# rpng/suo_slam

Hardware: AMD Instinct MI355X
Metric: frames/sec (obj-crops/sec) YCB-V 640x480 8-obj; ADD(-S) vs ref (higher is better)
Workload: dtype f32 (2 x fp16 split products)

## Files before the change

### suo_slam_amd/csrc/conv_wino_x3.hip

```cpp
#include <string.h>

#include "bf16x3.h"
#include "f16x2.h"
#include "buffer_ops.h"
#include "suo_internal.h"
#include "tune.h"

namespace suo {

typedef float x_f32x4 __attribute__((ext_vector_type(4)));
typedef float x_f32x16 __attribute__((ext_vector_type(16)));
typedef unsigned x_u32x2 __attribute__((ext_vector_type(2)));
typedef unsigned x_u32x4 __attribute__((ext_vector_type(4)));
typedef __bf16 x_bf16x8 __attribute__((ext_vector_type(8)));
typedef _Float16 x_f16x8 __attribute__((ext_vector_type(8)));

__device__ __forceinline__ x_f32x16 x_mfma32(float a, float b, x_f32x16 c) { return __builtin_amdgcn_mfma_f32_32x32x2f32(a, b, c, 0, 0, 0); }
__device__ __forceinline__ int x_acc_row(int r, int lane) { return (r & 3) + 8 * (r >> 2) + 4 * (lane >> 5); }

__device__ __forceinline__ x_f32x4 x_sub4(x_f32x4 a, x_f32x4 b) { return a - b; }
__device__ __forceinline__ x_f32x4 x_add4(x_f32x4 a, x_f32x4 b) { return a + b; }
__device__ __forceinline__ void x_add16(x_f32x16& z, const x_f32x16& t) { z += t; }
__device__ __forceinline__ void x_sub16(x_f32x16& z, const x_f32x16& t) { z -= t; }

constexpr int X_CK = 16, X_PKH = 20, X_TH = 8, X_TW = 16, X_IH = 10, X_IW = 18, X_NPIX = X_IH * X_IW;

void pack_wino_weight_bf16x3(const float* W, int N, int C, int Np, int Cp, const float* out_scale, uint16_t* out) {
    static const double G[4][3] = {{1, 0, 0}, {0.5, 0.5, 0.5}, {0.5, -0.5, 0.5}, {0, 0, 1}};
    const int NB = Np / 32;
    memset(out, 0, (size_t)Np * Cp * 16 * 3 * sizeof(uint16_t));
    for (int n = 0; n < N; ++n)
        for (int c = 0; c < C; ++c) {
            const float* g = W + ((size_t)n * C + c) * 9;
            const double sc = out_scale ? (double)out_scale[n] : 1.0;
            double Gg[4][3], U[4][4];
            for (int i = 0; i < 4; ++i)
                for (int j = 0; j < 3; ++j) Gg[i][j] = G[i][0] * g[j] + G[i][1] * g[3 + j] + G[i][2] * g[6 + j];
            for (int i = 0; i < 4; ++i)
                for (int j = 0; j < 4; ++j) U[i][j] = (Gg[i][0] * G[j][0] + Gg[i][1] * G[j][1] + Gg[i][2] * G[j][2]) * sc;
            const int chunk = c / X_CK, cc = c % X_CK, nb = n / 32, lane = (cc / 8) * 32 + (n % 32), e = cc % 8;
            for (int comp = 0; comp < 16; ++comp) {
                uint16_t t[3];
                s3_split_host((float)(comp >= 12 ? -U[comp >> 2][comp & 3] : U[comp >> 2][comp & 3]), t);
                for (int p = 0; p < 3; ++p) out[((((size_t)(chunk * 16 + comp) * NB + nb) * 3 + p) * 64 + lane) * 8 + e] = t[p];
            }
        }
}

void pack_tail_weight_bf16x3(const float* W3, int N2, int K, uint16_t* out) {
    const int NB = N2 / 32;
    for (int n = 0; n < N2; ++n)
        for (int k = 0; k < K; ++k) {
            const int ks = k / 16, kk = k % 16, lane = (kk / 8) * 32 + (n % 32), e = kk % 8, nb = n / 32;
            uint16_t t[3];
            s3_split_host(W3[(size_t)n * K + k], t);
            for (int p = 0; p < 3; ++p) out[((((size_t)(ks * NB + nb) * 3 + p) * 64 + lane) * 8) + e] = t[p];
        }
}

void pack_wino_weight_f16x2(const float* W, int N, int C, int Np, int Cp, const float* out_scale, uint16_t* out, float* oscale_out) {
    static const double G[4][3] = {{1, 0, 0}, {0.5, 0.5, 0.5}, {0.5, -0.5, 0.5}, {0, 0, 1}};
    const int NB = Np / 32;
    memset(out, 0, (size_t)Np * Cp * 16 * 2 * sizeof(uint16_t));
    for (int n = 0; n < Np; ++n) oscale_out[n] = ldexpf(1.f, -S2_XSHIFT);
    float* Un = (float*)malloc((size_t)C * 16 * sizeof(float));
    for (int n = 0; n < N; ++n) {
        float mx = 0.f;
        for (int c = 0; c < C; ++c) {
            const float* g = W + ((size_t)n * C + c) * 9;
            const double sc = out_scale ? (double)out_scale[n] : 1.0;
            double Gg[4][3];
            for (int i = 0; i < 4; ++i)
                for (int j = 0; j < 3; ++j) Gg[i][j] = G[i][0] * g[j] + G[i][1] * g[3 + j] + G[i][2] * g[6 + j];
            for (int i = 0; i < 4; ++i)
                for (int j = 0; j < 4; ++j) {
                    const float u = (float)((Gg[i][0] * G[j][0] + Gg[i][1] * G[j][1] + Gg[i][2] * G[j][2]) * sc);
                    Un[c * 16 + i * 4 + j] = i == 3 ? -u : u;
                    mx = fmaxf(mx, fabsf(u));
                }
        }
        const int t = s2_row_shift(mx);
        oscale_out[n] = ldexpf(1.f, -(t + S2_XSHIFT));
        for (int c = 0; c < C; ++c) {
            const int chunk = c / X_CK, cc = c % X_CK, nb = n / 32, lane = (cc / 8) * 32 + (n % 32), e = cc % 8;
            for (int comp = 0; comp < 16; ++comp) {
                uint16_t h[2];
                s2_split_host(ldexpf(Un[c * 16 + comp], t), h);
                for (int p = 0; p < 2; ++p) out[((((size_t)(chunk * 16 + comp) * NB + nb) * 2 + p) * 64 + lane) * 8 + e] = h[p];
            }
        }
    }
    free(Un);
}

void pack_tail_weight_f16x2(const float* W3, int N2, int K, uint16_t* out, float* oscale_out) { pack_gemm_weight_f16x2(W3, N2, K, out, oscale_out); }

template <bool FUSE, bool UP = false, bool TX3 = false, int NT = 4, int NP = 3, bool NEXT = false, bool W8 = false>
__global__ __launch_bounds__(W8 ? 512 : 256) __attribute__((amdgpu_waves_per_eu(2))) void wino3x3_x3_kernel(const ConvArgs a) {
    static_assert(NT == 4 || (NT == 2 && !FUSE), "64-channel form: plain convolution only");
    static_assert(!W8 || (NT == 4 && NP == 2 && !NEXT && (TX3 || !FUSE)), "eight waves: the fp16 form of the 128-channel kernel, without the next block's conv1");
    constexpr int NTHR = W8 ? 512 : 256;
    static_assert(!NEXT || (FUSE && TX3 && NP == 2), "the next block's conv1 rides on the fp16 tail");
    static_assert(NP == 3 || !FUSE || TX3, "the fp16 form's tail runs on the fp16 pipe");
    constexpr int HSZ = X_NPIX * X_PKH;
    constexpr int VROW = 16;
    constexpr int VPL = 16 * 32 * VROW;
    constexpr int VFLOATS = NP * VPL / 2;
    constexpr int TAILF = NP * 8 * (64 * 32 + 32) / 4;
    constexpr int SFLOATS = W8 ? (2 * HSZ + VFLOATS > TAILF + 8 * 32 * 36 ? 2 * HSZ + VFLOATS : TAILF + 8 * 32 * 36) : 2 * HSZ + VFLOATS;
    __shared__ __attribute__((aligned(16))) float S[SFLOATS];
    float (*Hin)[HSZ] = reinterpret_cast<float (*)[HSZ]>(&S[0]);
    uint16_t* V = reinterpret_cast<uint16_t*>(&S[2 * HSZ]);
    const int tid = threadIdx.x, lane = tid & 63;
    const int w = __builtin_amdgcn_readfirstlane(tid >> 6);
    const int tiles_x = (a.OW + X_TW - 1) / X_TW, tiles_y = (a.OH + X_TH - 1) / X_TH;
    int bid = blockIdx.x;
    if ((gridDim.x & 7) == 0) bid = (bid & 7) * (gridDim.x >> 3) + (bid >> 3);
    const int l = bid / (tiles_x * tiles_y);
    bid -= l * tiles_x * tiles_y;
    const int ty0 = bid / tiles_x, tx0 = bid - ty0 * tiles_x;
    const int oy0 = ty0 * X_TH, ox0 = tx0 * X_TW;
    const int iy0 = oy0 - 1, ix0 = ox0 - 1;
    const int nch = a.C / X_CK;
    const float* in_l = a.in + (size_t)l * a.H * a.W * a.C;
    const __amdgpu_buffer_rsrc_t in_srd = make_srd(in_l, (size_t)a.H * a.W * a.C * sizeof(float));
    const __amdgpu_buffer_rsrc_t w_srd = make_srd(a.Wp, (size_t)a.N * a.C * 16 * NP * sizeof(uint16_t));
    const __amdgpu_buffer_rsrc_t out_srd = make_srd(a.out + (size_t)l * a.OH * a.OW * a.N, (size_t)a.OH * a.OW * a.N * sizeof(float));

    constexpr int NF4 = X_NPIX * 4, NLD = (NF4 + NTHR - 1) / NTHR;
    int avoff[NLD];
#pragma unroll
    for (int i = 0; i < NLD; ++i) {
        const int idx = tid + i * NTHR;
        const int pix = idx >> 2, cc = idx & 3;
        const int py = pix / X_IW, px = pix - py * X_IW;
        const int iy = iy0 + py, ix = ix0 + px;
        const bool ok = idx < NF4 && iy >= 0 && iy < a.H && ix >= 0 && ix < a.W;
        avoff[i] = ok ? ((iy * a.W + ix) * a.C + cc * 4) * 4 : BUF_OOB;
    }
    x_f32x4 areg[NLD];
    auto gload = [&](int c) {
#pragma unroll
        for (int i = 0; i < NLD; ++i) areg[i] = buf_load(in_srd, avoff[i], c * X_CK * 4);
    };
    float dmax = 0.f;
    const float xs = NP == 2 ? s2_xscale(a.xscale) : 1.f;
    auto sstore = [&](int buf) {
#pragma unroll
        for (int i = 0; i < NLD; ++i) {
            const int idx = tid + i * NTHR;
            if constexpr (NP == 2) {
                areg[i] *= xs;
                dmax = s2_track(s2_track(dmax, areg[i][0], areg[i][1]), areg[i][2], areg[i][3]);
            }
            if (idx < NF4) *(x_f32x4*)&Hin[buf][(idx >> 2) * X_PKH + (idx & 3) * 4] = areg[i];
        }
    };
    const int wvoff = lane * 16;
    const int wn = NT == 4 ? (W8 ? (w & 3) : w) : (w & 1), wc = NT == 4 ? (W8 ? (w >> 2) : 0) : (w >> 1);
    constexpr bool HALF = NT == 2 || W8;
    constexpr int NPAIR = HALF ? 4 : 8;
    const int wsbase = wn * NP * 1024;
    auto bload = [&](int gc, x_u32x4 (&b)[NP]) {
        const int g = gc;
#pragma unroll
        for (int p = 0; p < NP; ++p) b[p] = __builtin_bit_cast(x_u32x4, buf_load(w_srd, wvoff + p * 1024, g * (NT * NP * 1024) + wsbase));
    };
    const int tt = tid & 31, tq = (tid >> 5) & 3, th = (tid >> 7) & 1;
    const int tv = __builtin_amdgcn_readfirstlane(tid >> 8);
    const int t_ty = tt >> 3, t_tx = tt & 7;
    const int hbase = ((2 * t_ty + th) * X_IW + 2 * t_tx) * X_PKH + tq * 4;
    const int vbase = tt * VROW + ((((tq >> 1) ^ (((tt >> 2) ^ (tt >> 3)) & 1)) * 8) + (tq & 1) * 4);
    auto vstore = [&](int comp, x_f32x4 v) {
        if constexpr (NP == 2) {
            const unsigned h0 = s2_pack_rn(v[0], v[1]), h1 = s2_pack_rn(v[2], v[3]);
            *(x_u32x2*)&V[comp * 32 * VROW + vbase] = x_u32x2{h0, h1};
            const unsigned l0 = s2_lo_pack(v[0], v[1], h0), l1 = s2_lo_pack(v[2], v[3], h1);
            *(x_u32x2*)&V[VPL + comp * 32 * VROW + vbase] = x_u32x2{l0, l1};
            return;
        }
#pragma unroll
        for (int p = 0; p < 3; ++p) {
            const unsigned q0 = s3_pack_rn(v[0], v[1]), q1 = s3_pack_rn(v[2], v[3]);
            *(x_u32x2*)&V[p * VPL + comp * 32 * VROW + vbase] = x_u32x2{q0, q1};
            if (p < 2) {
                v = x_sub4(v, x_f32x4{s3_lo(q0), s3_hi(q0), s3_lo(q1), s3_hi(q1)});
            }
        }
    };
    const int hother = th ? 0 : 2 * X_IW * X_PKH;
    const float hsign = th ? -1.f : 1.f;
    auto transform = [&](int buf) {
        const float* hs = &Hin[buf][hbase];
        if constexpr (W8) {
            const int xi = tv == 0 ? (th ? 3 : 0) : (th ? 2 : 1);
            x_f32x4 e[4];
#pragma unroll
            for (int c = 0; c < 4; ++c) {
                if (tv == 0) {
                    e[c] = x_sub4(*(const x_f32x4*)(hs + c * X_PKH), *(const x_f32x4*)(hs + (2 * X_IW + c) * X_PKH));
                } else {
                    const x_f32x4 l1 = *(const x_f32x4*)(hs + (X_IW + c) * X_PKH), lx = *(const x_f32x4*)(hs + hother + c * X_PKH);
                    e[c] = x_f32x4{__builtin_fmaf(lx[0], hsign, l1[0]), __builtin_fmaf(lx[1], hsign, l1[1]), __builtin_fmaf(lx[2], hsign, l1[2]), __builtin_fmaf(lx[3], hsign, l1[3])};
                }
            }
            vstore(xi * 4 + 0, x_sub4(e[0], e[2]));
            vstore(xi * 4 + 1, x_add4(e[1], e[2]));
            vstore(xi * 4 + 2, x_sub4(e[2], e[1]));
            vstore(xi * 4 + 3, x_sub4(e[1], e[3]));
            return;
        }
        x_f32x4 L0[4], L1[4], L2[4], Lx[4];
#pragma unroll
        for (int c = 0; c < 4; ++c) {
            L0[c] = *(const x_f32x4*)(hs + c * X_PKH);
            L1[c] = *(const x_f32x4*)(hs + (X_IW + c) * X_PKH);
            L2[c] = *(const x_f32x4*)(hs + (2 * X_IW + c) * X_PKH);
            Lx[c] = *(const x_f32x4*)(hs + hother + c * X_PKH);
        }
        x_f32x4 eA[4], eB[4];
#pragma unroll
        for (int c = 0; c < 4; ++c) {
            eA[c] = x_sub4(L0[c], L2[c]);
            eB[c] = x_f32x4{__builtin_fmaf(Lx[c][0], hsign, L1[c][0]), __builtin_fmaf(Lx[c][1], hsign, L1[c][1]), __builtin_fmaf(Lx[c][2], hsign, L1[c][2]),
                            __builtin_fmaf(Lx[c][3], hsign, L1[c][3])};
        }
        const int xiA = th ? 3 : 0, xiB = th ? 2 : 1;
        vstore(xiA * 4 + 0, x_sub4(eA[0], eA[2]));
        vstore(xiA * 4 + 1, x_add4(eA[1], eA[2]));
        vstore(xiA * 4 + 2, x_sub4(eA[2], eA[1]));
        vstore(xiA * 4 + 3, x_sub4(eA[1], eA[3]));
        vstore(xiB * 4 + 0, x_sub4(eB[0], eB[2]));
        vstore(xiB * 4 + 1, x_add4(eB[1], eB[2]));
        vstore(xiB * 4 + 2, x_sub4(eB[2], eB[1]));
        vstore(xiB * 4 + 3, x_sub4(eB[1], eB[3]));
    };

    x_f32x16 zero16;
#pragma unroll
    for (int r = 0; r < 16; ++r) zero16[r] = 0.f;
    x_f32x16 out[4], Z[8];
#pragma unroll
    for (int p = 0; p < 4; ++p)
#pragma unroll
        for (int r = 0; r < 16; ++r) out[p][r] = 0.f;
#pragma unroll
    for (int p = 0; p < 8; ++p)
#pragma unroll
        for (int r = 0; r < 16; ++r) Z[p][r] = 0.f;
    auto mac6 = [&](x_f32x16& acc, const x_bf16x8 (&f)[NP], const x_u32x4 (&bw)[NP], bool from_zero) {
        if constexpr (NP == 2) {
            constexpr int UI[3] = {0, 1, 0}, UJ[3] = {1, 0, 0};
#pragma unroll
            for (int t = 0; t < 3; ++t)
                acc = __builtin_amdgcn_mfma_f32_32x32x16_f16(__builtin_bit_cast(x_f16x8, f[UI[t]]), __builtin_bit_cast(x_f16x8, bw[UJ[t]]), (t == 0 && from_zero) ? zero16 : acc, 0, 0, 0);
            return;
        }
        constexpr int TI[6] = {0, 1, 2, 0, 1, 0}, TJ[6] = {2, 1, 0, 1, 0, 0};
#pragma unroll
        for (int t = 0; t < 6; ++t)
            acc = __builtin_amdgcn_mfma_f32_32x32x16_bf16(f[TI[t] % NP], __builtin_bit_cast(x_bf16x8, bw[TJ[t] % NP]), (t == 0 && from_zero) ? zero16 : acc, 0, 0, 0);
    };
    auto comp_of = [&](int pair, int which) -> int {
        if (!HALF) return pair < 4 ? (which ? 12 + pair : pair) : (which ? 8 + (pair - 4) : 4 + (pair - 4));
        return wc * 8 + 2 * pair + which;
    };
    const int afoff = (lane & 31) * VROW + (((lane >> 5) ^ (((lane >> 2) ^ (lane >> 3)) & 1)) * 8);
    x_u32x4 bring[2][2][NP];
    gload(0);
    bload(comp_of(0, 0), bring[0][0]);
    bload(comp_of(0, 1), bring[0][1]);
    sstore(0);
    __syncthreads();

#ifdef SUO_WX3_PROF
    long long pt[5] = {0, 0, 0, 0, 0}, p0 = clock64();
#define XPROF(i) do { const long long _t = clock64(); pt[i] += _t - p0; p0 = _t; } while (0)
#else
#define XPROF(i) do { } while (0)
#endif
    for (int c = 0; c < nch; ++c) {
        const int buf = c & 1;
        const bool more = c + 1 < nch;
        if (more) gload(c + 1);
        transform(buf);
        XPROF(0);
        __syncthreads();
        XPROF(1);
        if (more) sstore(buf ^ 1);
        XPROF(2);
#pragma unroll
        for (int pair = 0; pair < NPAIR; ++pair) {
            const int slot = pair & 1;
            {
                const int np = pair + 1 < NPAIR ? pair + 1 : 0, nc = pair + 1 < NPAIR ? c : (more ? c + 1 : c);
                bload(nc * 16 + comp_of(np, 0), bring[slot ^ 1][0]);
                bload(nc * 16 + comp_of(np, 1), bring[slot ^ 1][1]);
            }
            const int ca = comp_of(pair, 0), cb = comp_of(pair, 1);
            x_bf16x8 afa[NP], afb[NP];
#pragma unroll
            for (int p = 0; p < NP; ++p) {
                afa[p] = *(const x_bf16x8*)&V[p * VPL + ca * 32 * VROW + afoff];
                afb[p] = *(const x_bf16x8*)&V[p * VPL + cb * 32 * VROW + afoff];
            }
            __builtin_amdgcn_sched_barrier(0);
            if (HALF) {
                mac6(Z[2 * pair], afa, bring[slot][0], false);
                mac6(Z[2 * pair + 1], afb, bring[slot][1], false);
            } else if (pair < 4) {
                mac6(Z[pair], afa, bring[slot][0], false);
                mac6(Z[4 + pair], afb, bring[slot][1], false);
            } else {
                x_f32x16 ta, tb;
                mac6(ta, afa, bring[slot][0], true);
                mac6(tb, afb, bring[slot][1], true);
                x_add16(Z[pair - 4], ta); x_add16(Z[pair - 4], tb); x_add16(Z[pair], ta); x_sub16(Z[pair], tb);
            }
            __builtin_amdgcn_sched_barrier(0);
        }
        XPROF(3);
        __syncthreads();
        XPROF(4);
    }
#ifdef SUO_WX3_PROF
    if (blockIdx.x == 1000 && (tid & 63) == 0) printf("wave %d cycles: transform %lld  barrier1 %lld  sstore %lld  mfma+fold %lld  barrier2 %lld\n", w, pt[0], pt[1], pt[2], pt[3], pt[4]);
#endif
    if constexpr (NP == 2) s2_raise(a.range_flag, 4.f * dmax);
#pragma unroll
    for (int h = 0; h < 2; ++h) {
        out[2 * h] = Z[4 * h] + Z[4 * h + 1] + Z[4 * h + 2];
        out[2 * h + 1] = Z[4 * h + 1] - Z[4 * h + 2] - Z[4 * h + 3];
    }
    x_f32x16 mine[2];
    if constexpr (W8) {
        static_assert(VFLOATS >= 8 * 16 * 64, "the exchange area is the V planes");
        float* X = &S[2 * HSZ];
        const int pw = (1 - wc) * 4 + wn;
#pragma unroll
        for (int q = 0; q < 2; ++q) {
#pragma unroll
            for (int r = 0; r < 16; ++r) X[(w * 16 + r) * 64 + lane] = wc == 0 ? out[2 + q][r] : out[q][r];
            __syncthreads();
#pragma unroll
            for (int r = 0; r < 16; ++r) mine[q][r] = (wc == 0 ? out[q][r] + out[2 + q][r] : out[2 + q][r] - out[q][r]) + X[(pw * 16 + r) * 64 + lane];
            __syncthreads();
        }
    }

    if constexpr (FUSE && TX3) {
        constexpr int KS_STRIDE = 64 * 32 + 32;
        constexpr int PL_STRIDE = 8 * KS_STRIDE;
        static_assert(NP * PL_STRIDE == TAILF * 4 && NP * PL_STRIDE + (W8 ? 8 : 4) * 32 * 36 * 4 <= SFLOATS * 4, "tail staging must fit the workgroup's LDS");
        constexpr int NJ = W8 ? 1 : 2;
        unsigned char* AP = reinterpret_cast<unsigned char*>(&S[0]);
        float* T = &S[NP * PL_STRIDE / 4] + w * (32 * 36);
        const __amdgpu_buffer_rsrc_t w3_srd = make_srd(a.W3p, (size_t)a.N * a.N2 * NP * sizeof(uint16_t));
        const size_t crop2 = (size_t)a.OH * a.OW * a.N2;
        const __amdgpu_buffer_rsrc_t r_srd = make_srd(a.R + (size_t)l * crop2, crop2 * sizeof(float));
        const __amdgpu_buffer_rsrc_t o2_srd = make_srd(a.out2 + (size_t)l * crop2, crop2 * sizeof(float));
        constexpr bool has_up = UP;
        const __amdgpu_buffer_rsrc_t up_srd = make_srd(has_up ? a.up + (size_t)l * (crop2 / 4) : a.R, has_up ? crop2 / 4 * sizeof(float) : 0);
        const float xs3 = NP == 2 ? s2_xscale(a.xscale3) : 1.f;
        const float b2v = NP == 2 ? a.bias[wn * 32 + (lane & 31)] * xs3 : a.bias[wn * 32 + (lane & 31)];
        const float c2v = NP == 2 ? a.oscale[wn * 32 + (lane & 31)] * xs3 : 1.f;
        float tmax = 0.f;
        const int sbase = (2 * wn + ((lane >> 4) & 1)) * KS_STRIDE + (lane >> 5) * (8 * 32) + ((((lane >> 3) & 1) ^ (lane >> 5)) * 16) + (lane & 7) * 2;
        const int aoff = (lane & 31) * 32 + (((lane >> 5) ^ ((lane >> 3) & 1)) * 16);
        const int w3voff = lane * 16;
        auto b3load = [&](int ks, x_u32x4 (&b)[2][NP]) {
            const int k = ks < 8 ? ks : 7;
#pragma unroll
            for (int j = 0; j < NJ; ++j)
#pragma unroll
                for (int p = 0; p < NP; ++p) b[j][p] = __builtin_bit_cast(x_u32x4, buf_load(w3_srd, w3voff, (((k * 8 + (W8 ? w : 4 * j + w)) * NP) + p) * 1024));
        };
#pragma unroll
        for (int h = 0; h < 2; ++h) {
            x_u32x4 b3[2][2][NP];
            b3load(0, b3[0]);
            if (!W8 || wc == h)
#pragma unroll
            for (int pj = 0; pj < 2; ++pj)
#pragma unroll
                for (int r = 0; r < 16; ++r) {
                    const float cv = W8 ? mine[pj][r] : out[2 * h + pj][r];
                    float v = NP == 2 ? fmaxf(fmaf(cv, c2v, b2v), 0.f) : fmaxf(cv + b2v, 0.f);
                    const int off = sbase + (16 * (r >> 2) + 2 * (r & 3) + pj) * 32;
                    if constexpr (NP == 2) {
                        tmax = fmaxf(tmax, v);
                        const _Float16 hi = (_Float16)v, lo = (_Float16)(v - (float)hi);
                        *reinterpret_cast<_Float16*>(AP + off) = hi;
                        *reinterpret_cast<_Float16*>(AP + PL_STRIDE + off) = lo;
                        continue;
                    }
#pragma unroll
                    for (int p = 0; p < 3; ++p) {
                        const unsigned q = s3_pack_rn(v, v);
                        *reinterpret_cast<uint16_t*>(AP + p * PL_STRIDE + off) = (uint16_t)(q >> 16);
                        if (p < 2) v -= s3_hi(q);
                    }
                }
            __syncthreads();
            x_f32x16 acc2[2][2];
#pragma unroll
            for (int i = 0; i < 2; ++i)
#pragma unroll
                for (int j = 0; j < 2; ++j)
#pragma unroll
                    for (int r = 0; r < 16; ++r) acc2[i][j][r] = 0.f;
#pragma unroll
            for (int ks = 0; ks < 8; ++ks) {
                b3load(ks + 1, b3[(ks + 1) & 1]);
                x_bf16x8 af[2][NP];
#pragma unroll
                for (int i = 0; i < 2; ++i)
#pragma unroll
                    for (int p = 0; p < NP; ++p) af[i][p] = *(const x_bf16x8*)(AP + p * PL_STRIDE + ks * KS_STRIDE + i * 1024 + aoff);
                __builtin_amdgcn_sched_barrier(0);
#pragma unroll
                for (int i = 0; i < 2; ++i)
#pragma unroll
                    for (int j = 0; j < NJ; ++j) mac6(acc2[i][j], af[i], b3[ks & 1][j], false);
                __builtin_amdgcn_sched_barrier(0);
            }
            if constexpr (NEXT) __syncthreads();
            x_f32x16 acc1[2];
            if constexpr (NEXT) {
#pragma unroll
                for (int i = 0; i < 2; ++i) acc1[i] = zero16;
            }
#pragma unroll
            for (int j = 0; j < NJ; ++j) {
#pragma unroll
                for (int i = 0; i < 2; ++i) {
                    const int col = (W8 ? w : 4 * j + w) * 32 + (lane & 7) * 4;
                    const x_f32x4 bv = *(const x_f32x4*)(a.bias3 + col);
                    x_f32x4 osc3 = x_f32x4{1.f, 1.f, 1.f, 1.f};
                    if constexpr (NP == 2) osc3 = *(const x_f32x4*)(a.oscale3 + col);
                    x_f32x4 nsc, nsh;
                    if constexpr (NEXT) { const float nxs = s2_xscale(a.n_xscale); nsc = *(const x_f32x4*)(a.n_scale + col) * nxs; nsh = *(const x_f32x4*)(a.n_shift + col) * nxs; }
                    int off[4];
                    x_f32x4 rv[4], uv[UP ? 4 : 1];
#pragma unroll
                    for (int k = 0; k < 4; ++k) {
                        const int m = 32 * i + (lane >> 3) + 8 * k;
                        const int oy = oy0 + 2 * (m >> 4) + h, ox = ox0 + (m & 15);
                        const bool in = oy < a.OH && ox < a.OW;
                        off[k] = in ? ((oy * a.OW + ox) * a.N2 + col) * 4 : BUF_OOB;
                        rv[k] = buf_load(r_srd, off[k], 0);
                        if constexpr (UP && !NEXT) uv[k] = buf_load(up_srd, in ? (((oy >> 1) * (a.OW >> 1) + (ox >> 1)) * a.N2 + col) * 4 : BUF_OOB, 0);
                    }
#pragma unroll
                    for (int r = 0; r < 16; ++r) T[x_acc_row(r, lane) * 36 + (lane & 31)] = acc2[i][j][r];
                    __builtin_amdgcn_wave_barrier();
#pragma unroll
                    for (int k = 0; k < 4; ++k) {
                        if constexpr (UP && NEXT) {
                            const int m = 32 * i + (lane >> 3) + 8 * k;
                            const int oy = oy0 + 2 * (m >> 4) + h, ox = ox0 + (m & 15);
                            uv[0] = buf_load(up_srd, (oy < a.OH && ox < a.OW) ? (((oy >> 1) * (a.OW >> 1) + (ox >> 1)) * a.N2 + col) * 4 : BUF_OOB, 0);
                        }
                        x_f32x4 o = *(const x_f32x4*)&T[((lane >> 3) + 8 * k) * 36 + (lane & 7) * 4];
                        if constexpr (NP == 2) o *= osc3;
                        o = (o + bv) + rv[k];
                        if constexpr (UP) o += uv[NEXT ? 0 : k];
                        buf_store(o, o2_srd, off[k]);
                        if constexpr (NEXT) {
                            const int m = 32 * i + (lane >> 3) + 8 * k;
                            float xn[4];
#pragma unroll
                            for (int c = 0; c < 4; ++c) xn[c] = fmaxf(fmaf(o[c], nsc[c], nsh[c]), 0.f);
                            tmax = fmaxf(fmaxf(tmax, fmaxf(xn[0], xn[1])), fmaxf(xn[2], xn[3]));
                            const unsigned h0 = s2_pack_rn(xn[0], xn[1]), h1 = s2_pack_rn(xn[2], xn[3]);
                            const unsigned l0 = s2_lo_pack(xn[0], xn[1], h0), l1 = s2_lo_pack(xn[2], xn[3], h1);
                            unsigned char* d = AP + (2 * w + ((lane & 7) >> 2)) * KS_STRIDE + m * 32 + (((((lane & 3) >> 1) ^ ((m >> 3) & 1))) * 16) + (lane & 1) * 8;
                            *reinterpret_cast<x_u32x2*>(d) = x_u32x2{h0, h1};
                            *reinterpret_cast<x_u32x2*>(d + PL_STRIDE) = x_u32x2{l0, l1};
                        }
                    }
                    __builtin_amdgcn_wave_barrier();
                }
                if constexpr (NEXT) {
                    const __amdgpu_buffer_rsrc_t n1_srd = make_srd(a.n_W1, (size_t)128 * 256 * 2 * sizeof(uint16_t));
                    auto n1load = [&](int q, x_u32x4 (&b)[2]) {
                        const int ksg = 8 * j + (q < 8 ? q : 7);
#pragma unroll
                        for (int p = 0; p < 2; ++p) b[p] = __builtin_bit_cast(x_u32x4, buf_load(n1_srd, w3voff + p * 1024, ((ksg * 4 + w) * 2) * 1024));
                    };
                    constexpr int NR = 4;
                    x_u32x4 nb[NR][2];
#pragma unroll
                    for (int q = 0; q < NR - 1; ++q) n1load(q, nb[q]);
                    __syncthreads();
#pragma unroll
                    for (int q = 0; q < 8; ++q) {
                        n1load(q + NR - 1, nb[(q + NR - 1) % NR]);
                        x_bf16x8 af[2][2];
#pragma unroll
                        for (int i = 0; i < 2; ++i)
#pragma unroll
                            for (int p = 0; p < 2; ++p) af[i][p] = *(const x_bf16x8*)(AP + p * PL_STRIDE + q * KS_STRIDE + i * 1024 + aoff);
                        __builtin_amdgcn_sched_barrier(0);
#pragma unroll
                        for (int i = 0; i < 2; ++i) mac6(acc1[i], af[i], nb[q % NR], false);
                        __builtin_amdgcn_sched_barrier(0);
                    }
                    __syncthreads();
                }
            }
            if constexpr (NEXT) {
                const int col = w * 32 + (lane & 7) * 4;
                const x_f32x4 b1 = *(const x_f32x4*)(a.n_b1 + col), o1 = *(const x_f32x4*)(a.n_osc1 + col);
                const size_t cropn = (size_t)a.OH * a.OW * 128;
                const __amdgpu_buffer_rsrc_t n_srd = make_srd(a.n_out + (size_t)l * cropn, cropn * sizeof(float));
#pragma unroll
                for (int i = 0; i < 2; ++i) {
#pragma unroll
                    for (int r = 0; r < 16; ++r) T[x_acc_row(r, lane) * 36 + (lane & 31)] = acc1[i][r];
                    __builtin_amdgcn_wave_barrier();
#pragma unroll
                    for (int k = 0; k < 4; ++k) {
                        const int m = 32 * i + (lane >> 3) + 8 * k;
                        const int oy = oy0 + 2 * (m >> 4) + h, ox = ox0 + (m & 15);
                        x_f32x4 o = *(const x_f32x4*)&T[((lane >> 3) + 8 * k) * 36 + (lane & 7) * 4];
                        o *= o1;
                        o += b1;
#pragma unroll
                        for (int c = 0; c < 4; ++c) o[c] = fmaxf(o[c], 0.f);
                        buf_store(o, n_srd, (oy < a.OH && ox < a.OW) ? ((oy * a.OW + ox) * 128 + col) * 4 : BUF_OOB);
                    }
                    __builtin_amdgcn_wave_barrier();
                }
            }
            if (h == 0 && !NEXT) __syncthreads();
        }
        if constexpr (NP == 2) s2_raise(a.range_flag, tmax);
        return;
    }

    if constexpr (FUSE && !TX3) {
        constexpr int MP = 132;
        static_assert(128 * MP <= 2 * HSZ + VFLOATS, "the conv2 tile must fit the workgroup's LDS");
        float* M2 = &S[0];
        const int wm = w >> 1, wn = w & 1;
        const int NB2 = a.N2 >> 5;
        const __amdgpu_buffer_rsrc_t w3_srd = make_srd(a.W3p, (size_t)a.N * a.N2 * sizeof(float));
        const size_t crop2 = (size_t)a.OH * a.OW * a.N2;
        const __amdgpu_buffer_rsrc_t r_srd = make_srd(a.R + (size_t)l * crop2, crop2 * sizeof(float));
        const __amdgpu_buffer_rsrc_t o2_srd = make_srd(a.out2 + (size_t)l * crop2, crop2 * sizeof(float));
        constexpr bool has_up = UP;
        const __amdgpu_buffer_rsrc_t up_srd = make_srd(has_up ? a.up + (size_t)l * (crop2 / 4) : a.R, has_up ? crop2 / 4 * sizeof(float) : 0);
        const float b2v = a.bias[w * 32 + (lane & 31)];
        const int w3voff = lane * 16;
        auto b3load = [&](int q, x_f32x4(&b)[4]) {
            const int kg = q < 16 ? q : 15;
#pragma unroll
            for (int j = 0; j < 4; ++j) b[j] = buf_load(w3_srd, w3voff, (kg * NB2 + wn * 4 + j) * 1024);
        };
        constexpr int R3 = 3;
        x_f32x4 b3[R3][4];
#pragma unroll
        for (int r = 0; r < R3 - 1; ++r) b3load(r, b3[r]);
#pragma unroll
        for (int p = 0; p < 4; ++p)
#pragma unroll
            for (int r = 0; r < 16; ++r) {
                const int t = x_acc_row(r, lane);
                const int pix = (2 * (t >> 3) + (p >> 1)) * X_TW + 2 * (t & 7) + (p & 1);
                M2[pix * MP + w * 32 + (lane & 31)] = fmaxf(out[p][r] + b2v, 0.f);
            }
        __syncthreads();
        x_f32x16 acc2[2][4];
#pragma unroll
        for (int i = 0; i < 2; ++i)
#pragma unroll
            for (int j = 0; j < 4; ++j)
#pragma unroll
                for (int r = 0; r < 16; ++r) acc2[i][j][r] = 0.f;
        const float* ms = M2 + ((wm * 2) * 32 + (lane & 31)) * MP + (lane >> 5) * 4;
#pragma unroll
        for (int q = 0; q < 16; ++q) {
            b3load(q + R3 - 1, b3[(q + R3 - 1) % R3]);
            __builtin_amdgcn_sched_barrier(0);
            x_f32x4 af[2];
#pragma unroll
            for (int i = 0; i < 2; ++i) af[i] = *(const x_f32x4*)(ms + i * 32 * MP + q * 8);
#pragma unroll
            for (int t = 0; t < 4; ++t)
#pragma unroll
                for (int i = 0; i < 2; ++i)
#pragma unroll
                    for (int j = 0; j < 4; ++j) acc2[i][j] = x_mfma32(af[i][t], b3[q % R3][j][t], acc2[i][j]);
            __builtin_amdgcn_sched_barrier(0);
        }
        __syncthreads();
#pragma unroll
        for (int i = 0; i < 2; ++i)
#pragma unroll
            for (int j = 0; j < 4; ++j) {
                float* T = M2 + w * (32 * 36);
                const int col = (wn * 4 + j) * 32 + (lane & 7) * 4;
                const x_f32x4 bv = *(const x_f32x4*)(a.bias3 + col);
                int off[4];
                x_f32x4 rv[4], uv[UP ? 4 : 1];
#pragma unroll
                for (int k = 0; k < 4; ++k) {
                    const int pp = (wm * 2 + i) * 32 + (lane >> 3) + 8 * k;
                    const int oy = oy0 + pp / X_TW, ox = ox0 + pp % X_TW;
                    const bool in = oy < a.OH && ox < a.OW;
                    off[k] = in ? ((oy * a.OW + ox) * a.N2 + col) * 4 : BUF_OOB;
                    rv[k] = buf_load(r_srd, off[k], 0);
                    if constexpr (UP) uv[k] = buf_load(up_srd, in ? (((oy >> 1) * (a.OW >> 1) + (ox >> 1)) * a.N2 + col) * 4 : BUF_OOB, 0);
                }
#pragma unroll
                for (int r = 0; r < 16; ++r) T[x_acc_row(r, lane) * 36 + (lane & 31)] = acc2[i][j][r];
                __builtin_amdgcn_wave_barrier();
#pragma unroll
                for (int k = 0; k < 4; ++k) {
                    x_f32x4 o = (*(const x_f32x4*)&T[((lane >> 3) + 8 * k) * 36 + (lane & 7) * 4] + bv) + rv[k];
                    if constexpr (UP) o += uv[k];
                    buf_store(o, o2_srd, off[k]);
                }
                __builtin_amdgcn_wave_barrier();
            }
        return;
    }

    if constexpr (NT == 2 || W8) {
        if constexpr (NT == 2) {
            float* X = &S[2 * HSZ];
#pragma unroll
            for (int q = 0; q < 2; ++q)
#pragma unroll
                for (int r = 0; r < 16; ++r) X[((w * 2 + q) * 16 + r) * 64 + lane] = wc == 0 ? out[2 + q][r] : out[q][r];
            __syncthreads();
            const int pw = (1 - wc) * 2 + wn;
#pragma unroll
            for (int q = 0; q < 2; ++q)
#pragma unroll
                for (int r = 0; r < 16; ++r)
                    mine[q][r] = (wc == 0 ? out[q][r] + out[2 + q][r] : out[2 + q][r] - out[q][r]) + X[((pw * 2 + q) * 16 + r) * 64 + lane];
            __syncthreads();
        }
        float* T = &S[2 * HSZ] + w * (32 * 36);
        const int col = wn * 32 + (lane & 7) * 4;
        const x_f32x4 bv = *(const x_f32x4*)(a.bias + col);
        x_f32x4 osc = x_f32x4{1.f, 1.f, 1.f, 1.f};
        if constexpr (NP == 2) osc = *(const x_f32x4*)(a.oscale + col);
#pragma unroll
        for (int q = 0; q < 2; ++q) {
            const int p = 2 * wc + q, pi = p >> 1, pj = p & 1;
#pragma unroll
            for (int r = 0; r < 16; ++r) T[x_acc_row(r, lane) * 36 + (lane & 31)] = mine[q][r];
            __builtin_amdgcn_wave_barrier();
#pragma unroll
            for (int k = 0; k < 4; ++k) {
                const int t = (lane >> 3) + 8 * k;
                const int oy = oy0 + 2 * (t >> 3) + pi, ox = ox0 + 2 * (t & 7) + pj;
                x_f32x4 o = *(const x_f32x4*)&T[t * 36 + (lane & 7) * 4];
                if constexpr (NP == 2) o *= osc;
                o += bv;
                if (a.relu) {
#pragma unroll
                    for (int z = 0; z < 4; ++z) o[z] = fmaxf(o[z], 0.f);
                }
                buf_store(o, out_srd, (oy < a.OH && ox < a.OW) ? ((oy * a.OW + ox) * a.N + col) * 4 : BUF_OOB);
            }
            __builtin_amdgcn_wave_barrier();
        }
        return;
    }

    float* T = &S[2 * HSZ] + w * (32 * 36);
    const int col = w * 32 + (lane & 7) * 4;
    const x_f32x4 bv = *(const x_f32x4*)(a.bias + col);
    x_f32x4 osc = x_f32x4{1.f, 1.f, 1.f, 1.f};
    if constexpr (NP == 2) osc = *(const x_f32x4*)(a.oscale + col);
#pragma unroll
    for (int p = 0; p < 4; ++p) {
        const int pi = p >> 1, pj = p & 1;
#pragma unroll
        for (int r = 0; r < 16; ++r) T[x_acc_row(r, lane) * 36 + (lane & 31)] = out[p][r];
        __builtin_amdgcn_wave_barrier();
#pragma unroll
        for (int k = 0; k < 4; ++k) {
            const int t = (lane >> 3) + 8 * k;
            const int oy = oy0 + 2 * (t >> 3) + pi, ox = ox0 + 2 * (t & 7) + pj;
            x_f32x4 o = *(const x_f32x4*)&T[t * 36 + (lane & 7) * 4];
            if constexpr (NP == 2) o *= osc;
            o += bv;
            if (a.relu) {
#pragma unroll
                for (int q = 0; q < 4; ++q) o[q] = fmaxf(o[q], 0.f);
            }
            buf_store(o, out_srd, (oy < a.OH && ox < a.OW) ? ((oy * a.OW + ox) * a.N + col) * 4 : BUF_OOB);
        }
        __builtin_amdgcn_wave_barrier();
    }
}

bool conv3x3_wino_f16x2_w8(long tiles) {
    static const long upto = SUO_TUNE("SUO_WINO_W8_TILES", 256);
    return tiles > 0 && tiles <= upto && env_switch("SUO_WINO_W8", 1) != 0;
}

template <int NP>
static int launch_wino_split(const ConvArgs& a, hipStream_t s) {
    if (NP == 2 && (!a.oscale || !a.range_flag)) { suo_set_error("conv3x3_wino_f16x2: oscale / range_flag missing"); return SUO_ERR_ARG; }
    if (a.OH == a.H && a.OW == a.W && a.N == 64 && a.C == 64) {
        const int tiles64 = ((a.OW + X_TW - 1) / X_TW) * ((a.OH + X_TH - 1) / X_TH) * a.L;
        hipLaunchKernelGGL((wino3x3_x3_kernel<false, false, false, 2, NP>), dim3(tiles64), dim3(256), 0, s, a);
        SUO_HIP_CHECK(hipGetLastError());
        return SUO_OK;
    }
    if (a.OH != a.H || a.OW != a.W || a.N != 128 || a.C != 128) {
        suo_set_error("conv3x3_wino_x3: unsupported shape H=%d W=%d C=%d N=%d", a.H, a.W, a.C, a.N);
        return SUO_ERR_ARG;
    }
    const int tiles = ((a.OW + X_TW - 1) / X_TW) * ((a.OH + X_TH - 1) / X_TH) * a.L;
    if (NP == 2 && conv3x3_wino_f16x2_w8(tiles)) hipLaunchKernelGGL((wino3x3_x3_kernel<false, false, false, 4, 2, false, true>), dim3(tiles), dim3(512), 0, s, a);
    else hipLaunchKernelGGL((wino3x3_x3_kernel<false, false, false, 4, NP>), dim3(tiles), dim3(256), 0, s, a);
    SUO_HIP_CHECK(hipGetLastError());
    return SUO_OK;
}
int launch_conv3x3_wino_x3(const ConvArgs& a, hipStream_t s) { return launch_wino_split<3>(a, s); }
int launch_conv3x3_wino_f16x2(const ConvArgs& a, hipStream_t s) { return launch_wino_split<2>(a, s); }

int launch_conv3x3_wino_f16x2_fused(const ConvArgs& a, hipStream_t s) {
    if (a.OH != a.H || a.OW != a.W || a.N != 128 || a.C != 128 || a.N2 != 256 || !a.W3p || !a.bias3 || !a.R || !a.out2 || !a.oscale || !a.oscale3 || !a.range_flag) {
        suo_set_error("conv3x3_wino_f16x2_fused: unsupported shape C=%d N=%d N2=%d", a.C, a.N, a.N2);
        return SUO_ERR_ARG;
    }
    const int tiles = ((a.OW + X_TW - 1) / X_TW) * ((a.OH + X_TH - 1) / X_TH) * a.L;
    if (a.n_W1) {
        if (!a.n_scale || !a.n_shift || !a.n_osc1 || !a.n_b1 || !a.n_out) { suo_set_error("conv3x3_wino_f16x2_fused: incomplete next-block arguments"); return SUO_ERR_ARG; }
        if (a.up) { suo_set_error("conv3x3_wino_f16x2_fused: the next block's conv1 cannot ride on a tail with an up-sampled addend"); return SUO_ERR_ARG; }
        hipLaunchKernelGGL((wino3x3_x3_kernel<true, false, true, 4, 2, true>), dim3(tiles), dim3(256), 0, s, a);
    } else if (conv3x3_wino_f16x2_w8(tiles)) {
        if (a.up) hipLaunchKernelGGL((wino3x3_x3_kernel<true, true, true, 4, 2, false, true>), dim3(tiles), dim3(512), 0, s, a);
        else hipLaunchKernelGGL((wino3x3_x3_kernel<true, false, true, 4, 2, false, true>), dim3(tiles), dim3(512), 0, s, a);
    } else if (a.up) hipLaunchKernelGGL((wino3x3_x3_kernel<true, true, true, 4, 2>), dim3(tiles), dim3(256), 0, s, a);
    else hipLaunchKernelGGL((wino3x3_x3_kernel<true, false, true, 4, 2>), dim3(tiles), dim3(256), 0, s, a);
    SUO_HIP_CHECK(hipGetLastError());
    return SUO_OK;
}

int launch_conv3x3_wino_x3_fused(const ConvArgs& a, hipStream_t s) {
    if (a.OH != a.H || a.OW != a.W || a.N != 128 || a.C != 128 || a.N2 != 256 || !a.W3p || !a.bias3 || !a.R || !a.out2) {
        suo_set_error("conv3x3_wino_x3_fused: unsupported shape C=%d N=%d N2=%d", a.C, a.N, a.N2);
        return SUO_ERR_ARG;
    }
    const int tiles = ((a.OW + X_TW - 1) / X_TW) * ((a.OH + X_TH - 1) / X_TH) * a.L;
    if (a.w3_bf16x3) {
        if (a.up) hipLaunchKernelGGL((wino3x3_x3_kernel<true, true, true>), dim3(tiles), dim3(256), 0, s, a);
        else hipLaunchKernelGGL((wino3x3_x3_kernel<true, false, true>), dim3(tiles), dim3(256), 0, s, a);
    } else {
        if (a.up) hipLaunchKernelGGL((wino3x3_x3_kernel<true, true, false>), dim3(tiles), dim3(256), 0, s, a);
        else hipLaunchKernelGGL((wino3x3_x3_kernel<true, false, false>), dim3(tiles), dim3(256), 0, s, a);
    }
    SUO_HIP_CHECK(hipGetLastError());
    return SUO_OK;
}

}
```

Measured before the change: 1377.

## Stage the upsampled skip tile in LDS once per workgroup for the fp16 tail

For the fused fp16 tail with an upsample input, each wave now loads its share of the half-resolution skip tile into registers early and writes it to LDS once. The epilogue then reads the skip values from LDS instead of issuing a scattered global load per output pixel for each of the two row halves. The per-wave transpose patch is halved and processed in two passes so the extra LDS fits under a two-workgroups-per-CU budget. This trades extra LDS use, additional wave barriers and early register pressure for fewer redundant global reads of the upsample tensor.

```diff
diff --git a/suo_slam_amd/csrc/conv_wino_x3.hip b/suo_slam_amd/csrc/conv_wino_x3.hip
--- a/suo_slam_amd/csrc/conv_wino_x3.hip
+++ b/suo_slam_amd/csrc/conv_wino_x3.hip
@@ -107,7 +107,14 @@
     constexpr int VPL = 16 * 32 * VROW;
     constexpr int VFLOATS = NP * VPL / 2;
     constexpr int TAILF = NP * 8 * (64 * 32 + 32) / 4;
-    constexpr int SFLOATS = W8 ? (2 * HSZ + VFLOATS > TAILF + 8 * 32 * 36 ? 2 * HSZ + VFLOATS : TAILF + 8 * 32 * 36) : 2 * HSZ + VFLOATS;
+    constexpr bool UPL = FUSE && UP && TX3 && NP == 2;
+    constexpr int NW = W8 ? 8 : 4;
+    constexpr int TQ = UPL && !W8 ? 2 : 1;
+    constexpr int TPATCH = 32 * 36 / TQ;
+    constexpr int UPF = UPL ? 32 * 256 : 0;
+    constexpr int SBASE = W8 ? (2 * HSZ + VFLOATS > TAILF + 8 * 32 * 36 ? 2 * HSZ + VFLOATS : TAILF + 8 * 32 * 36) : 2 * HSZ + VFLOATS;
+    constexpr int SFLOATS = UPL && TAILF + NW * TPATCH + UPF > SBASE ? TAILF + NW * TPATCH + UPF : SBASE;
+    static_assert(W8 || SFLOATS * 4 <= 80 * 1024, "two workgroups per CU");
     __shared__ __attribute__((aligned(16))) float S[SFLOATS];
     float (*Hin)[HSZ] = reinterpret_cast<float (*)[HSZ]>(&S[0]);
     uint16_t* V = reinterpret_cast<uint16_t*>(&S[2 * HSZ]);
@@ -351,16 +358,27 @@
     if constexpr (FUSE && TX3) {
         constexpr int KS_STRIDE = 64 * 32 + 32;
         constexpr int PL_STRIDE = 8 * KS_STRIDE;
-        static_assert(NP * PL_STRIDE == TAILF * 4 && NP * PL_STRIDE + (W8 ? 8 : 4) * 32 * 36 * 4 <= SFLOATS * 4, "tail staging must fit the workgroup's LDS");
+        static_assert(NP * PL_STRIDE == TAILF * 4 && NP * PL_STRIDE + (NW * TPATCH + UPF) * 4 <= SFLOATS * 4, "tail staging must fit the workgroup's LDS");
         constexpr int NJ = W8 ? 1 : 2;
         unsigned char* AP = reinterpret_cast<unsigned char*>(&S[0]);
-        float* T = &S[NP * PL_STRIDE / 4] + w * (32 * 36);
+        float* T = &S[NP * PL_STRIDE / 4] + w * TPATCH;
         const __amdgpu_buffer_rsrc_t w3_srd = make_srd(a.W3p, (size_t)a.N * a.N2 * NP * sizeof(uint16_t));
         const size_t crop2 = (size_t)a.OH * a.OW * a.N2;
         const __amdgpu_buffer_rsrc_t r_srd = make_srd(a.R + (size_t)l * crop2, crop2 * sizeof(float));
         const __amdgpu_buffer_rsrc_t o2_srd = make_srd(a.out2 + (size_t)l * crop2, crop2 * sizeof(float));
         constexpr bool has_up = UP;
         const __amdgpu_buffer_rsrc_t up_srd = make_srd(has_up ? a.up + (size_t)l * (crop2 / 4) : a.R, has_up ? crop2 / 4 * sizeof(float) : 0);
+        constexpr int NU = UPL ? 32 / NW : 1;
+        float* UW = &S[NP * PL_STRIDE / 4 + NW * TPATCH] + w * (UPF / NW);
+        x_f32x4 ust[NU];
+        if constexpr (UPL) {
+            const int lx = (ox0 >> 1) + (lane >> 3);
+#pragma unroll
+            for (int q = 0; q < NU; ++q) {
+                const int ly = (oy0 >> 1) + (q & 3), colq = (W8 ? w : 4 * (q >> 2) + w) * 32 + (lane & 7) * 4;
+                ust[q] = buf_load(up_srd, (2 * ly < a.OH && 2 * lx < a.OW) ? ((ly * (a.OW >> 1) + lx) * a.N2 + colq) * 4 : BUF_OOB, 0);
+            }
+        }
         const float xs3 = NP == 2 ? s2_xscale(a.xscale3) : 1.f;
         const float b2v = NP == 2 ? a.bias[wn * 32 + (lane & 31)] * xs3 : a.bias[wn * 32 + (lane & 31)];
         const float c2v = NP == 2 ? a.oscale[wn * 32 + (lane & 31)] * xs3 : 1.f;
@@ -401,6 +419,12 @@
                         if (p < 2) v -= s3_hi(q);
                     }
                 }
+            if constexpr (UPL) {
+                if (h == 0) {
+#pragma unroll
+                    for (int q = 0; q < NU; ++q) *(x_f32x4*)&UW[(q * 64 + lane) * 4] = ust[q];
+                }
+            }
             __syncthreads();
             x_f32x16 acc2[2][2];
 #pragma unroll
@@ -441,7 +465,7 @@
                     x_f32x4 nsc, nsh;
                     if constexpr (NEXT) { const float nxs = s2_xscale(a.n_xscale); nsc = *(const x_f32x4*)(a.n_scale + col) * nxs; nsh = *(const x_f32x4*)(a.n_shift + col) * nxs; }
                     int off[4];
-                    x_f32x4 rv[4], uv[UP ? 4 : 1];
+                    x_f32x4 rv[4], uv[UP && !UPL ? 4 : 1];
 #pragma unroll
                     for (int k = 0; k < 4; ++k) {
                         const int m = 32 * i + (lane >> 3) + 8 * k;
@@ -449,37 +473,37 @@
                         const bool in = oy < a.OH && ox < a.OW;
                         off[k] = in ? ((oy * a.OW + ox) * a.N2 + col) * 4 : BUF_OOB;
                         rv[k] = buf_load(r_srd, off[k], 0);
-                        if constexpr (UP && !NEXT) uv[k] = buf_load(up_srd, in ? (((oy >> 1) * (a.OW >> 1) + (ox >> 1)) * a.N2 + col) * 4 : BUF_OOB, 0);
+                        if constexpr (UP && !UPL) uv[k] = buf_load(up_srd, in ? (((oy >> 1) * (a.OW >> 1) + (ox >> 1)) * a.N2 + col) * 4 : BUF_OOB, 0);
                     }
 #pragma unroll
-                    for (int r = 0; r < 16; ++r) T[x_acc_row(r, lane) * 36 + (lane & 31)] = acc2[i][j][r];
-                    __builtin_amdgcn_wave_barrier();
-#pragma unroll
-                    for (int k = 0; k < 4; ++k) {
-                        if constexpr (UP && NEXT) {
-                            const int m = 32 * i + (lane >> 3) + 8 * k;
-                            const int oy = oy0 + 2 * (m >> 4) + h, ox = ox0 + (m & 15);
-                            uv[0] = buf_load(up_srd, (oy < a.OH && ox < a.OW) ? (((oy >> 1) * (a.OW >> 1) + (ox >> 1)) * a.N2 + col) * 4 : BUF_OOB, 0);
+                    for (int tq = 0; tq < TQ; ++tq) {
+#pragma unroll
+                        for (int r = tq * (16 / TQ); r < (tq + 1) * (16 / TQ); ++r) T[(x_acc_row(r, lane) - tq * 16) * 36 + (lane & 31)] = acc2[i][j][r];
+                        __builtin_amdgcn_wave_barrier();
+#pragma unroll
+                        for (int k = tq * (4 / TQ); k < (tq + 1) * (4 / TQ); ++k) {
+                            x_f32x4 o = *(const x_f32x4*)&T[((lane >> 3) + 8 * k - tq * 16) * 36 + (lane & 7) * 4];
+                            if constexpr (NP == 2) o *= osc3;
+                            o = (o + bv) + rv[k];
+                            if constexpr (UPL) {
+                                o += *(const x_f32x4*)&UW[((4 * j + 2 * i + (k >> 1)) * 64 + ((lane >> 4) + 4 * (k & 1)) * 8 + (lane & 7)) * 4];
+                            } else if constexpr (UP) o += uv[k];
+                            buf_store(o, o2_srd, off[k]);
+                            if constexpr (NEXT) {
+                                const int m = 32 * i + (lane >> 3) + 8 * k;
+                                float xn[4];
+#pragma unroll
+                                for (int c = 0; c < 4; ++c) xn[c] = fmaxf(fmaf(o[c], nsc[c], nsh[c]), 0.f);
+                                tmax = fmaxf(fmaxf(tmax, fmaxf(xn[0], xn[1])), fmaxf(xn[2], xn[3]));
+                                const unsigned h0 = s2_pack_rn(xn[0], xn[1]), h1 = s2_pack_rn(xn[2], xn[3]);
+                                const unsigned l0 = s2_lo_pack(xn[0], xn[1], h0), l1 = s2_lo_pack(xn[2], xn[3], h1);
+                                unsigned char* d = AP + (2 * w + ((lane & 7) >> 2)) * KS_STRIDE + m * 32 + (((((lane & 3) >> 1) ^ ((m >> 3) & 1))) * 16) + (lane & 1) * 8;
+                                *reinterpret_cast<x_u32x2*>(d) = x_u32x2{h0, h1};
+                                *reinterpret_cast<x_u32x2*>(d + PL_STRIDE) = x_u32x2{l0, l1};
+                            }
                         }
-                        x_f32x4 o = *(const x_f32x4*)&T[((lane >> 3) + 8 * k) * 36 + (lane & 7) * 4];
-                        if constexpr (NP == 2) o *= osc3;
-                        o = (o + bv) + rv[k];
-                        if constexpr (UP) o += uv[NEXT ? 0 : k];
-                        buf_store(o, o2_srd, off[k]);
-                        if constexpr (NEXT) {
-                            const int m = 32 * i + (lane >> 3) + 8 * k;
-                            float xn[4];
-#pragma unroll
-                            for (int c = 0; c < 4; ++c) xn[c] = fmaxf(fmaf(o[c], nsc[c], nsh[c]), 0.f);
-                            tmax = fmaxf(fmaxf(tmax, fmaxf(xn[0], xn[1])), fmaxf(xn[2], xn[3]));
-                            const unsigned h0 = s2_pack_rn(xn[0], xn[1]), h1 = s2_pack_rn(xn[2], xn[3]);
-                            const unsigned l0 = s2_lo_pack(xn[0], xn[1], h0), l1 = s2_lo_pack(xn[2], xn[3], h1);
-                            unsigned char* d = AP + (2 * w + ((lane & 7) >> 2)) * KS_STRIDE + m * 32 + (((((lane & 3) >> 1) ^ ((m >> 3) & 1))) * 16) + (lane & 1) * 8;
-                            *reinterpret_cast<x_u32x2*>(d) = x_u32x2{h0, h1};
-                            *reinterpret_cast<x_u32x2*>(d + PL_STRIDE) = x_u32x2{l0, l1};
-                        }
+                        __builtin_amdgcn_wave_barrier();
                     }
-                    __builtin_amdgcn_wave_barrier();
                 }
                 if constexpr (NEXT) {
                     const __amdgpu_buffer_rsrc_t n1_srd = make_srd(a.n_W1, (size_t)128 * 256 * 2 * sizeof(uint16_t));
@@ -517,20 +541,23 @@
 #pragma unroll
                 for (int i = 0; i < 2; ++i) {
 #pragma unroll
-                    for (int r = 0; r < 16; ++r) T[x_acc_row(r, lane) * 36 + (lane & 31)] = acc1[i][r];
-                    __builtin_amdgcn_wave_barrier();
-#pragma unroll
-                    for (int k = 0; k < 4; ++k) {
-                        const int m = 32 * i + (lane >> 3) + 8 * k;
-                        const int oy = oy0 + 2 * (m >> 4) + h, ox = ox0 + (m & 15);
-                        x_f32x4 o = *(const x_f32x4*)&T[((lane >> 3) + 8 * k) * 36 + (lane & 7) * 4];
-                        o *= o1;
-                        o += b1;
-#pragma unroll
-                        for (int c = 0; c < 4; ++c) o[c] = fmaxf(o[c], 0.f);
-                        buf_store(o, n_srd, (oy < a.OH && ox < a.OW) ? ((oy * a.OW + ox) * 128 + col) * 4 : BUF_OOB);
+                    for (int tq = 0; tq < TQ; ++tq) {
+#pragma unroll
+                        for (int r = tq * (16 / TQ); r < (tq + 1) * (16 / TQ); ++r) T[(x_acc_row(r, lane) - tq * 16) * 36 + (lane & 31)] = acc1[i][r];
+                        __builtin_amdgcn_wave_barrier();
+#pragma unroll
+                        for (int k = tq * (4 / TQ); k < (tq + 1) * (4 / TQ); ++k) {
+                            const int m = 32 * i + (lane >> 3) + 8 * k;
+                            const int oy = oy0 + 2 * (m >> 4) + h, ox = ox0 + (m & 15);
+                            x_f32x4 o = *(const x_f32x4*)&T[((lane >> 3) + 8 * k - tq * 16) * 36 + (lane & 7) * 4];
+                            o *= o1;
+                            o += b1;
+#pragma unroll
+                            for (int c = 0; c < 4; ++c) o[c] = fmaxf(o[c], 0.f);
+                            buf_store(o, n_srd, (oy < a.OH && ox < a.OW) ? ((oy * a.OW + ox) * 128 + col) * 4 : BUF_OOB);
+                        }
+                        __builtin_amdgcn_wave_barrier();
                     }
-                    __builtin_amdgcn_wave_barrier();
                 }
             }
             if (h == 0 && !NEXT) __syncthreads();
```

New measurement: 1381, median of 4. Within noise of the previous version (+0.3%).
